# summa-dev/circuits-halo2

Hardware: AMD Instinct MI355X
Metric: msm_points_per_sec (higher is better)
Workload: dtype u32; 1 GPU; standalone BN254 G1 MSM, 2^20 uniform Fr scalars x synthetic-SRS affine points per GPU (BASELINE configs[1]); points_per_gpu=1048576, steps_in_flight=3

## Files before the change

### circuits_halo2_amd/csrc/bn254_curve29.cuh

```cuda
#pragma once
#include "bn254_f29.cuh"

#ifndef SG_FUSED_Y3
#define SG_FUSED_Y3 1
#endif

namespace sg {

struct affine29 {
  f29 x, y;
  bool inf;
};
struct xyzz29 {
  f29 x, y, zz, zzz;
};

SG_HD bool xyzz29_is_identity(const xyzz29& p) { return f29_all_zero(p.zz); }
SG_HD xyzz29 xyzz29_identity() {
  xyzz29 r;
  r.x = f29_zero();
  r.y = f29_zero();
  r.zz = f29_zero();
  r.zzz = f29_zero();
  return r;
}

SG_HD affine29 affine29_from_words(const uint32_t w[16]) {
  affine29 r;
  uint32_t o = 0;
#pragma unroll
  for (int i = 0; i < 16; i++) o |= w[i];
  r.inf = (o == 0);
  r.x = f29_from_words<5>(w);
  r.y = f29_from_words<5>(w + 8);
  return r;
}
SG_HD void affine29_negate(affine29& q) { q.y = f29_sub<Fq29, 4>(f29_zero(), q.y); }

SG_HD xyzz29 xyzz29_double_affine(const affine29& q) {
  typedef Fq29 P;
  if (q.inf) return xyzz29_identity();
  xyzz29 r;
  f29 x = f29_mul<P>(q.x, f29_one<P>());
  f29 y = f29_mul<P>(q.y, f29_one<P>());
  f29 u = f29_dbl(y);
  f29 v = f29_sqr<P>(u);
  f29 w = f29_mul<P>(u, v);
  f29 s = f29_mul<P>(x, v);
  f29 xx = f29_sqr<P>(x);
  f29 m = f29_add(f29_dbl(xx), xx);
  r.x = f29_sub<P, 1>(f29_sqr<P>(m), f29_dbl(s));
  f29 t = f29_sub<P, 2>(s, r.x);
#if SG_FUSED_Y3
  r.y = f29_mul2<P>(m, t, w, f29_sub<P, 0>(f29_zero(), y));
#else
  r.y = f29_sub<P, 0>(f29_mul<P>(m, t), f29_mul<P>(w, y));
#endif
  r.zz = v;
  r.zzz = w;
  return r;
}
SG_HD xyzz29 xyzz29_double(const xyzz29& p) {
  typedef Fq29 P;
  if (xyzz29_is_identity(p)) return p;
  xyzz29 r;
  f29 u = f29_dbl(p.y);
  f29 v = f29_sqr<P>(u);
  f29 w = f29_mul<P>(u, v);
  f29 s = f29_mul<P>(p.x, v);
  f29 xx = f29_sqr<P>(p.x);
  f29 m = f29_add(f29_dbl(xx), xx);
  r.x = f29_sub<P, 1>(f29_sqr<P>(m), f29_dbl(s));
  f29 t = f29_sub<P, 2>(s, r.x);
#if SG_FUSED_Y3
  r.y = f29_mul2<P>(m, t, w, f29_sub<P, 1>(f29_zero(), p.y));
#else
  r.y = f29_sub<P, 0>(f29_mul<P>(m, t), f29_mul<P>(w, p.y));
#endif
  r.zz = f29_mul<P>(v, p.zz);
  r.zzz = f29_mul<P>(w, p.zzz);
  return r;
}

SG_HD void xyzz29_madd(xyzz29& acc, const affine29& q) {
  typedef Fq29 P;
  if (q.inf) return;
  if (xyzz29_is_identity(acc)) {
    acc.x = f29_mul<P>(q.x, f29_one<P>());
    acc.y = f29_mul<P>(q.y, f29_one<P>());
    acc.zz = f29_one<P>();
    acc.zzz = f29_one<P>();
    return;
  }
  f29 u2 = f29_mul<P>(q.x, acc.zz);
  f29 s2 = f29_mul<P>(q.y, acc.zzz);
  f29 p = f29_sub<P, 2>(u2, acc.x);
  f29 r = f29_sub<P, 1>(s2, acc.y);
  if (f29_is_zero_mod_p<P>(p)) {
    if (f29_is_zero_mod_p<P>(r)) acc = xyzz29_double_affine(q);
    else acc = xyzz29_identity();
    return;
  }
  f29 pp = f29_sqr<P>(p);
  f29 ppp = f29_mul<P>(p, pp);
  f29 qq = f29_mul<P>(acc.x, pp);
  f29 rr = f29_sqr<P>(r);
  f29 x3 = f29_carry(f29_sub_nc<P, 1>(f29_sub_nc<P, 0>(rr, ppp), f29_add_nc(qq, qq)));
  f29 t = f29_carry_top(f29_sub_nc<P, 2>(qq, x3));
#if SG_FUSED_Y3
  f29 y3 = f29_mul2<P>(t, r, f29_sub<P, 1>(f29_zero(), acc.y), ppp);
#else
  f29 y3 = f29_sub<P, 0>(f29_mul<P>(t, r), f29_mul<P>(acc.y, ppp));
#endif
  acc.zz = f29_mul<P>(acc.zz, pp);
  acc.zzz = f29_mul<P>(acc.zzz, ppp);
  acc.x = x3;
  acc.y = y3;
}

SG_HD void xyzz29_add(xyzz29& acc, const xyzz29& q) {
  typedef Fq29 P;
  if (xyzz29_is_identity(q)) return;
  if (xyzz29_is_identity(acc)) {
    acc = q;
    return;
  }
  f29 u1 = f29_mul<P>(acc.x, q.zz);
  f29 u2 = f29_mul<P>(q.x, acc.zz);
  f29 s1 = f29_mul<P>(acc.y, q.zzz);
  f29 s2 = f29_mul<P>(q.y, acc.zzz);
  f29 p = f29_sub<P, 0>(u2, u1);
  f29 r = f29_sub<P, 0>(s2, s1);
  if (f29_is_zero_mod_p<P>(p)) {
    if (f29_is_zero_mod_p<P>(r)) acc = xyzz29_double(acc);
    else acc = xyzz29_identity();
    return;
  }
  f29 pp = f29_sqr<P>(p);
  f29 ppp = f29_mul<P>(p, pp);
  f29 qq = f29_mul<P>(u1, pp);
  f29 rr = f29_sqr<P>(r);
  f29 x3 = f29_carry(f29_sub_nc<P, 1>(f29_sub_nc<P, 0>(rr, ppp), f29_add_nc(qq, qq)));
  f29 t = f29_carry_top(f29_sub_nc<P, 2>(qq, x3));
#if SG_FUSED_Y3
  f29 y3 = f29_mul2<P>(t, r, f29_sub<P, 0>(f29_zero(), s1), ppp);
#else
  f29 y3 = f29_sub<P, 0>(f29_mul<P>(t, r), f29_mul<P>(s1, ppp));
#endif
  acc.zz = f29_mul<P>(f29_mul<P>(acc.zz, q.zz), pp);
  acc.zzz = f29_mul<P>(f29_mul<P>(acc.zzz, q.zzz), ppp);
  acc.x = x3;
  acc.y = y3;
}

SG_HD void xyzz29_to_words(const xyzz29& p, uint32_t w[32]) {
  typedef Fq29 P;
  f29_to_words(f29_reduce_with<P>(p.x, P::r256), w);
  f29_to_words(f29_reduce_with<P>(p.y, P::r256), w + 8);
  f29_to_words(f29_reduce_with<P>(p.zz, P::r256), w + 16);
  f29_to_words(f29_reduce_with<P>(p.zzz, P::r256), w + 24);
}

}

#if defined(__HIPCC__)
namespace sg {
struct alignas(16) g1_affine_mem {
  uint4 q[4];
};
struct alignas(16) xyzz29_mem {
  uint4 q[9];
};
struct alignas(16) fp_words {
  uint4 q[2];
};

__device__ __forceinline__ affine29 affine29_load(const g1_affine_mem* p) {
  uint32_t w[16];
#pragma unroll
  for (int i = 0; i < 4; i++) {
    uint4 v = p->q[i];
    w[4 * i] = v.x; w[4 * i + 1] = v.y; w[4 * i + 2] = v.z; w[4 * i + 3] = v.w;
  }
  return affine29_from_words(w);
}
__device__ __forceinline__ xyzz29 xyzz29_load(const xyzz29_mem* p) {
  uint32_t w[36];
#pragma unroll
  for (int i = 0; i < 9; i++) {
    uint4 v = p->q[i];
    w[4 * i] = v.x; w[4 * i + 1] = v.y; w[4 * i + 2] = v.z; w[4 * i + 3] = v.w;
  }
  xyzz29 r;
#pragma unroll
  for (int i = 0; i < 9; i++) { r.x.l[i] = w[i]; r.y.l[i] = w[9 + i]; r.zz.l[i] = w[18 + i]; r.zzz.l[i] = w[27 + i]; }
  return r;
}
__device__ __forceinline__ void xyzz29_store(xyzz29_mem* p, const xyzz29& v) {
  uint32_t w[36];
#pragma unroll
  for (int i = 0; i < 9; i++) { w[i] = v.x.l[i]; w[9 + i] = v.y.l[i]; w[18 + i] = v.zz.l[i]; w[27 + i] = v.zzz.l[i]; }
#pragma unroll
  for (int i = 0; i < 9; i++) p->q[i] = make_uint4(w[4 * i], w[4 * i + 1], w[4 * i + 2], w[4 * i + 3]);
}
__device__ __forceinline__ void fp_words_load(const fp_words* p, uint32_t w[8]) {
  uint4 a = p->q[0], b = p->q[1];
  w[0] = a.x; w[1] = a.y; w[2] = a.z; w[3] = a.w; w[4] = b.x; w[5] = b.y; w[6] = b.z; w[7] = b.w;
}
__device__ __forceinline__ void fp_words_store(fp_words* p, const uint32_t w[8]) {
  p->q[0] = make_uint4(w[0], w[1], w[2], w[3]);
  p->q[1] = make_uint4(w[4], w[5], w[6], w[7]);
}
template <class P>
__device__ inline f29 f29_inv(const f29& x) {
  return f29_inv_safegcd<P>(x);
}
template <class P>
__device__ inline f29 f29_pow_u64(f29 x, uint64_t e) {
  f29 acc = f29_one<P>();
  while (e) {
    if (e & 1) acc = f29_mul<P>(acc, x);
    x = f29_sqr<P>(x);
    e >>= 1;
  }
  return acc;
}
template <class P>
__device__ __forceinline__ f29 f29_load_r256(const fp_words* p) {
  uint32_t w[8];
  fp_words_load(p, w);
  return f29_from_words<0>(w);
}
template <class P>
__device__ __forceinline__ f29 f29_words_to_r261(const uint32_t w[8]) {
  f29 k;
#pragma unroll
  for (int i = 0; i < 9; i++) k.l[i] = P::r266[i];
  return f29_mul<P>(f29_from_words<0>(w), k);
}
template <class P>
__device__ __forceinline__ void f29_store_canonical(fp_words* p, const f29& a_lt2p_normalised) {
  uint32_t w[8];
  f29_to_words(f29_cond_sub_p<P>(a_lt2p_normalised), w);
  fp_words_store(p, w);
}
template <int SRC>
__device__ __forceinline__ f29 quad_bcast(const f29& v) {
  f29 r;
#pragma unroll
  for (int i = 0; i < 9; i++) {
    int t = __builtin_amdgcn_mov_dpp((int)v.l[i], SRC * 0x55, 0xf, 0xf, true);
    asm volatile("" : "+v"(t));
    r.l[i] = (uint32_t)t;
  }
  return r;
}
__device__ __forceinline__ f29 quad_sel(uint32_t role, const f29& a0, const f29& a1, const f29& a2, const f29& a3) {
  f29 r;
#pragma unroll
  for (int i = 0; i < 9; i++) {
    uint32_t lo = (role & 1) ? a1.l[i] : a0.l[i];
    uint32_t hi = (role & 1) ? a3.l[i] : a2.l[i];
    r.l[i] = (role & 2) ? hi : lo;
  }
  return r;
}
__device__ __forceinline__ void xyzz29_add_quad(xyzz29& acc, const xyzz29& q, uint32_t role) {
  typedef Fq29 P;
  if (xyzz29_is_identity(q)) return;
  if (xyzz29_is_identity(acc)) {
    acc = q;
    return;
  }
  f29 m = f29_mul<P>(quad_sel(role, acc.x, q.x, acc.y, q.y), quad_sel(role, q.zz, acc.zz, q.zzz, acc.zzz));
  const f29 u1 = quad_bcast<0>(m), u2 = quad_bcast<1>(m), s1 = quad_bcast<2>(m), s2 = quad_bcast<3>(m);
  const f29 p = f29_sub<P, 0>(u2, u1);
  const f29 r = f29_sub<P, 0>(s2, s1);
  if (f29_is_zero_mod_p<P>(p)) {
    if (f29_is_zero_mod_p<P>(r)) acc = xyzz29_double(acc);
    else acc = xyzz29_identity();
    return;
  }
  m = f29_mul<P>(quad_sel(role, p, r, acc.zz, acc.zzz), quad_sel(role, p, r, q.zz, q.zzz));
  const f29 pp = quad_bcast<0>(m), rr = quad_bcast<1>(m);
  m = f29_mul<P>(quad_sel(role, p, u1, m, m), quad_sel(role, pp, pp, pp, p));
  const f29 ppp = quad_bcast<0>(m), qq = quad_bcast<1>(m), zz3 = quad_bcast<2>(m);
  const f29 x3 = f29_carry(f29_sub_nc<P, 1>(f29_sub_nc<P, 0>(rr, ppp), f29_add_nc(qq, qq)));
  const f29 t = f29_carry_top(f29_sub_nc<P, 2>(qq, x3));
  m = f29_mul<P>(quad_sel(role, t, s1, s1, m), quad_sel(role, r, ppp, ppp, pp));
  acc.y = f29_sub<P, 0>(quad_bcast<0>(m), quad_bcast<1>(m));
  acc.zzz = quad_bcast<3>(m);
  acc.zz = zz3;
  acc.x = x3;
}
}
#endif
```

### circuits_halo2_amd/csrc/msm_accumulate.cuh

```cuda
#pragma once
#include "msm.h"
#include "side_prio.cuh"

namespace sg {

__device__ __forceinline__ uint32_t find_owner(const uint32_t* __restrict__ toff, uint32_t NB, uint32_t t) {
  uint32_t lo = 0, hi = NB;
  while (hi - lo > 1) {
    uint32_t mid = (lo + hi) >> 1;
    if (toff[mid] <= t) lo = mid; else hi = mid;
  }
  return lo;
}

__global__ void __launch_bounds__(256) msm_accumulate(const uint32_t* __restrict__ sorted, BatchPtrs bp,
                                                      uint32_t buckets_per_msm,
                                                      const uint32_t* __restrict__ off,
                                                      const uint32_t* __restrict__ cnt,
                                                      const uint32_t* __restrict__ toff,
                                                      const uint2* __restrict__ order, uint32_t log_L,
                                                      const uint32_t* __restrict__ meta, uint32_t* __restrict__ ticket,
                                                      xyzz29_mem* __restrict__ partial, uint64_t* __restrict__ trace) {
  const uint32_t ntasks = meta[1], lane = threadIdx.x & 63u;
  const uint32_t wave_id = (blockIdx.x * blockDim.x + threadIdx.x) >> 6;
  if (trace && lane == 0) trace[2 * wave_id] = wall_clock64();
  for (;;) {
    uint32_t base = 0;
    if (lane == 0) base = atomicAdd(ticket, 64u);
    base = __builtin_amdgcn_readfirstlane(base);
    if (base >= ntasks) break;
    const uint32_t t = base + lane;
    if (t < ntasks) {
      const uint2 o = order[t];
      const uint32_t b = o.x, seg = o.y;
      const g1_affine_mem* __restrict__ bases = bp.bases[b / buckets_per_msm];
      uint32_t start = off[b] + (seg << log_L);
      uint32_t end = min(off[b] + cnt[b], start + (1u << log_L));
      xyzz29 acc = xyzz29_identity();
      uint32_t e = sorted[start];
      g1_affine_mem raw = bases[e & 0x7fffffffu];
      for (uint32_t k = start; k < end; k++) {
        uint32_t e_next = 0;
        g1_affine_mem raw_next = raw;
        if (k + 1 < end) {
          e_next = sorted[k + 1];
          raw_next = bases[e_next & 0x7fffffffu];
        }
        affine29 p = affine29_load(&raw);
        if (e >> 31) affine29_negate(p);
        xyzz29_madd(acc, p);
        e = e_next;
        raw = raw_next;
      }
      xyzz29_store(partial + toff[b] + seg, acc);
    }
  }
  if (trace && lane == 0) trace[2 * wave_id + 1] = wall_clock64();
}

template <int Q>
__device__ __forceinline__ void add_q(xyzz29& acc, const xyzz29& q, uint32_t role) {
  if (Q == 4) xyzz29_add_quad(acc, q, role);
  else xyzz29_add(acc, q);
}
template <int Q>
__global__ void __launch_bounds__(256) msm_merge(const xyzz29_mem* __restrict__ in, const uint32_t* __restrict__ off,
                                                 const uint32_t* __restrict__ cnt, const uint32_t* __restrict__ toff,
                                                 uint32_t NB, uint32_t log_L, const uint32_t* __restrict__ meta,
                                                 xyzz29_mem* __restrict__ out) {
  side_kernel_prio();
  const uint32_t t = (blockIdx.x * blockDim.x + threadIdx.x) / Q, role = threadIdx.x % Q;
  if (t >= meta[1]) return;
  uint32_t b = find_owner(toff, NB, t);
  uint32_t seg = t - toff[b];
  uint32_t start = off[b] + (seg << log_L);
  uint32_t end = min(off[b] + cnt[b], start + (1u << log_L));
  xyzz29 acc = xyzz29_identity();
  for (uint32_t k = start; k < end; k++) add_q<Q>(acc, xyzz29_load(in + k), role);
  if (role == 0) xyzz29_store(out + t, acc);
}

}
```

Baseline: 820.7 million points/s.

## Make bucket accumulation branch-free with optimistic ordinary madd and fallback redo

The per-thread bucket accumulation loop now runs an unconditional ordinary mixed addition. It folds the sign negation into the r computation and records whether any infinity or equal/opposite-point case occurred; if one did, the segment is recomputed with the fully checked madd. The first two points are combined with an affine+affine add (mmadd) that yields zz=pp and zzz=ppp directly, skipping the identity-initialisation step. This removes warp divergence and per-iteration identity/special-case branches in the hot loop. The cost is extra register pressure and a rare full recompute of the segment.

```diff
diff --git a/circuits_halo2_amd/csrc/bn254_curve29.cuh b/circuits_halo2_amd/csrc/bn254_curve29.cuh
--- a/circuits_halo2_amd/csrc/bn254_curve29.cuh
+++ b/circuits_halo2_amd/csrc/bn254_curve29.cuh
@@ -116,6 +116,94 @@
   acc.zzz = f29_mul<P>(acc.zzz, ppp);
   acc.x = x3;
   acc.y = y3;
+}
+
+SG_HD xyzz29 xyzz29_from_affine(const affine29& q) {
+  typedef Fq29 P;
+  if (q.inf) return xyzz29_identity();
+  xyzz29 r;
+  r.x = f29_reduce_small<P>(q.x);
+  r.y = f29_reduce_small<P>(f29_normalize(q.y));
+  r.zz = f29_one<P>();
+  r.zzz = f29_one<P>();
+  return r;
+}
+
+SG_HD int xyzz29_madd_ordinary(xyzz29& acc, const affine29& q, bool neg) {
+  typedef Fq29 P;
+  f29 u2 = f29_mul<P>(q.x, acc.zz);
+  f29 s2 = f29_mul<P>(q.y, acc.zzz);
+  f29 p = f29_sub<P, 2>(u2, acc.x);
+  const uint32_t mask = neg ? 0xffffffffu : 0u;
+  f29 r;
+#pragma unroll
+  for (int i = 0; i < 9; i++)
+    r.l[i] = ((s2.l[i] ^ mask) + (P::subc[1][i] - acc.y.l[i])) + (mask & (P::subc[2][i] - P::subc[1][i] + 1u));
+  r = f29_carry(r);
+  int special = 0;
+  if (f29_is_zero_mod_p<P>(p)) special = f29_is_zero_mod_p<P>(r) ? 2 : 1;
+  f29 pp = f29_sqr<P>(p);
+  f29 ppp = f29_mul<P>(p, pp);
+  f29 qq = f29_mul<P>(acc.x, pp);
+  f29 rr = f29_sqr<P>(r);
+  f29 x3 = f29_carry(f29_sub_nc<P, 1>(f29_sub_nc<P, 0>(rr, ppp), f29_add_nc(qq, qq)));
+  f29 t = f29_carry_top(f29_sub_nc<P, 2>(qq, x3));
+#if SG_FUSED_Y3
+  f29 y3 = f29_mul2<P>(t, r, f29_sub<P, 1>(f29_zero(), acc.y), ppp);
+#else
+  f29 y3 = f29_sub<P, 0>(f29_mul<P>(t, r), f29_mul<P>(acc.y, ppp));
+#endif
+  acc.zz = f29_mul<P>(acc.zz, pp);
+  acc.zzz = f29_mul<P>(acc.zzz, ppp);
+  acc.x = x3;
+  acc.y = y3;
+  return special;
+}
+SG_HD void xyzz29_madd(xyzz29& acc, const affine29& q, bool neg) {
+  if (q.inf) return;
+  affine29 s = q;
+  if (neg) affine29_negate(s);
+  if (xyzz29_is_identity(acc)) {
+    acc = xyzz29_from_affine(s);
+    return;
+  }
+  xyzz29 sum = acc;
+  const int special = xyzz29_madd_ordinary(sum, q, neg);
+  if (special == 0) acc = sum;
+  else if (special == 2) acc = xyzz29_double_affine(s);
+  else acc = xyzz29_identity();
+}
+
+SG_HD int xyzz29_mmadd_ordinary(xyzz29& out, const affine29& a, const affine29& b) {
+  typedef Fq29 P;
+  f29 p = f29_reduce_small<P>(f29_sub<P, 5>(b.x, a.x));
+  f29 r = f29_reduce_small<P>(f29_sub<P, 5>(b.y, a.y));
+  int special = 0;
+  if (f29_is_zero_mod_p<P>(p)) special = f29_is_zero_mod_p<P>(r) ? 2 : 1;
+  f29 pp = f29_sqr<P>(p);
+  f29 ppp = f29_mul<P>(p, pp);
+  f29 qq = f29_mul<P>(a.x, pp);
+  f29 rr = f29_sqr<P>(r);
+  f29 x3 = f29_carry(f29_sub_nc<P, 1>(f29_sub_nc<P, 0>(rr, ppp), f29_add_nc(qq, qq)));
+  f29 t = f29_carry_top(f29_sub_nc<P, 2>(qq, x3));
+#if SG_FUSED_Y3
+  out.y = f29_mul2<P>(t, r, f29_sub<P, 5>(f29_zero(), a.y), ppp);
+#else
+  out.y = f29_sub<P, 0>(f29_mul<P>(t, r), f29_mul<P>(a.y, ppp));
+#endif
+  out.x = x3;
+  out.zz = pp;
+  out.zzz = ppp;
+  return special;
+}
+SG_HD xyzz29 xyzz29_mmadd(const affine29& a, const affine29& b) {
+  if (a.inf) return xyzz29_from_affine(b);
+  if (b.inf) return xyzz29_from_affine(a);
+  xyzz29 r;
+  const int special = xyzz29_mmadd_ordinary(r, a, b);
+  if (special == 2) return xyzz29_double_affine(a);
+  if (special == 1) return xyzz29_identity();
+  return r;
 }
 
 SG_HD void xyzz29_add(xyzz29& acc, const xyzz29& q) {
diff --git a/circuits_halo2_amd/csrc/msm_accumulate.cuh b/circuits_halo2_amd/csrc/msm_accumulate.cuh
--- a/circuits_halo2_amd/csrc/msm_accumulate.cuh
+++ b/circuits_halo2_amd/csrc/msm_accumulate.cuh
@@ -11,6 +11,16 @@
     if (toff[mid] <= t) lo = mid; else hi = mid;
   }
   return lo;
+}
+
+__device__ __forceinline__ affine29 affine29_take(const g1_affine_mem& raw, bool& redo) {
+  affine29 p = affine29_load(&raw);
+  uint32_t inf = p.inf;
+#pragma unroll
+  for (int i = 0; i < 9; i++) asm volatile("" : "+v"(p.x.l[i]), "+v"(p.y.l[i]));
+  asm volatile("" : "+v"(inf) : : "memory");
+  redo |= inf != 0;
+  return p;
 }
 
 __global__ void __launch_bounds__(256) msm_accumulate(const uint32_t* __restrict__ sorted, BatchPtrs bp,
@@ -36,21 +46,37 @@
       const g1_affine_mem* __restrict__ bases = bp.bases[b / buckets_per_msm];
       uint32_t start = off[b] + (seg << log_L);
       uint32_t end = min(off[b] + cnt[b], start + (1u << log_L));
-      xyzz29 acc = xyzz29_identity();
-      uint32_t e = sorted[start];
-      g1_affine_mem raw = bases[e & 0x7fffffffu];
-      for (uint32_t k = start; k < end; k++) {
-        uint32_t e_next = 0;
-        g1_affine_mem raw_next = raw;
-        if (k + 1 < end) {
-          e_next = sorted[k + 1];
-          raw_next = bases[e_next & 0x7fffffffu];
+      const uint32_t last = max(end, start + 1) - 1;
+      uint32_t e = sorted[start], e1 = sorted[min(start + 1, last)];
+      g1_affine_mem raw = bases[e & 0x7fffffffu], raw1 = bases[e1 & 0x7fffffffu];
+      bool redo = end <= start;
+      affine29 p0 = affine29_take(raw, redo);
+      if (e >> 31) affine29_negate(p0);
+      xyzz29 acc;
+      uint32_t k = start + 2;
+      if (end - start == 1) {
+        acc = xyzz29_from_affine(p0);
+      } else {
+        affine29 p1 = affine29_take(raw1, redo);
+        if (e1 >> 31) affine29_negate(p1);
+        e = sorted[min(k, last)];
+        raw = bases[e & 0x7fffffffu];
+        redo |= xyzz29_mmadd_ordinary(acc, p0, p1) != 0;
+      }
+      for (; k < end; k++) {
+        const affine29 p = affine29_take(raw, redo);
+        const bool neg = e >> 31;
+        e = sorted[min(k + 1, last)];
+        raw = bases[e & 0x7fffffffu];
+        redo |= xyzz29_madd_ordinary(acc, p, neg) != 0;
+      }
+      if (redo) {
+        acc = xyzz29_identity();
+        for (uint32_t i = start; i < end; i++) {
+          const uint32_t ei = sorted[i];
+          const g1_affine_mem q = bases[ei & 0x7fffffffu];
+          xyzz29_madd(acc, affine29_load(&q), ei >> 31);
         }
-        affine29 p = affine29_load(&raw);
-        if (e >> 31) affine29_negate(p);
-        xyzz29_madd(acc, p);
-        e = e_next;
-        raw = raw_next;
       }
       xyzz29_store(partial + toff[b] + seg, acc);
     }
```

Result: faster. 841.3 million points/s, median of 6 (+2.5%).
